# JADGardner/neusky

Hardware: AMD Instinct MI355X
Metric: train rays/sec on NeRF-OSR lk2 @1024 rays x 96 samples (higher is better)
Workload: dtype f32 in memory; forward products: fp16 hi + residual split, 3 x v_mfma_f32_32x32x16_f16 per product on power-of-two pre-scaled operands, one fp32 accumulator (~2^-22): FiLM-SIREN chains and the SDF / albedo field alike; backward products: the same fp16 split on per-row / per-matrix pre-scaled gradien; 1 GPU; full NeuSky train step (BASELINE configs[2]): 1024 rays/GPU x 96 samples, proposal 256+96, 512 illumination directions (256 upper-hemisphere DDF queries/ray), illumination decoder = this project's FiLM-SIREN H = 128 (RENI-shaped: latent 100x3; the reference's configured Attention decoder is absent from its tree), hash L16 F2 T2^19 x2, 256-wide MLPs; fwd + losses + bwd + all-reduce + 5 Adam groups; rays_per_gpu=1024, samples_per_ray=96, illumination_directions=512, parallelism=ray-sharded dp1, launcher=self-spawned, launch=HIP graph replay (1 graph/step + all-reduce + 5 Adam launches)

## Files before the change

### neusky_amd/csrc/field_chain.hip

```cpp
#include "chain.h"

namespace {

constexpr int H = 256, NT = 8, KS = 16;
constexpr int WAVES = 4, PW = 16 / WAVES, RG = WAVES == 8 ? 8 : 4, RING = RG * GROUP, THREADS = 64 * WAVES, WGS_PER_CU = 8 / WAVES;

struct ChainLayers { nsky_chain_layer l[NSKY_CHAIN_MAX_LAYERS]; int n; };

__host__ __device__ inline void chain_layout(const nsky_chain_layer* l, int n, long& groups, int& tiles) {
  groups = 0; tiles = 0;
  for (int i = 0; i < n; ++i) {
    const int t = (l[i].rows + 31) / 32;
    tiles += t;
    groups += (long)t * groups_of(l[i].K);
  }
}

__global__ __launch_bounds__(256) void chain_pack_kernel(ChainLayers L, unsigned char* __restrict__ stream, float* __restrict__ scales) {
  __shared__ float w[32][PACK_KMAX + 1];
  __shared__ float red[256];
  int tile = blockIdx.x, i = 0;
  long group = 0;
  for (; i < L.n; ++i) {
    const int t = (L.l[i].rows + 31) / 32;
    if (tile < t) break;
    tile -= t;
    group += (long)t * groups_of(L.l[i].K);
  }
  const nsky_chain_layer& y = L.l[i];
  TileDesc d;
  d.W = y.W; d.ld = y.ld; d.row0 = 32 * tile; d.nrows = min(32, y.rows - 32 * tile); d.K = y.K; d.transposed = y.transposed; d.k0 = 0;
  d.group = group + (long)tile * groups_of(y.K);
  pack_tile(d, stream, scales, w, red);
}

template <int G>
__device__ __forceinline__ float quad_bcast(float v) {
  return __int_as_float(__builtin_amdgcn_mov_dpp(__float_as_int(v), G * 0x55, 0xf, 0xf, true));
}
__device__ __forceinline__ float quad_bcast0(float v) { return quad_bcast<0>(v); }
__device__ __forceinline__ float quad_sum(float v) {
  v += __int_as_float(__builtin_amdgcn_mov_dpp(__float_as_int(v), 0xB1, 0xf, 0xf, true));
  v += __int_as_float(__builtin_amdgcn_mov_dpp(__float_as_int(v), 0x4E, 0xf, 0xf, true));
  return v;
}
__device__ __forceinline__ float quad_max(float v) {
  v = fmaxf(v, __int_as_float(__builtin_amdgcn_mov_dpp(__float_as_int(v), 0xB1, 0xf, 0xf, true)));
  v = fmaxf(v, __int_as_float(__builtin_amdgcn_mov_dpp(__float_as_int(v), 0x4E, 0xf, 0xf, true)));
  return v;
}
__device__ __forceinline__ void quad_scatter_value(const float (&x)[16], int j, float (&mine)[4]) {
#pragma unroll
// ... 625 lines not shown
  }
  for (int u = 0; u < ct; ++u) {
    f32x16 acc;
    prod<KS, PW, true, RG>(ws, ACTIVE, ph, pl, acc);
    if (ACTIVE && live && a.dET) {
      const float inv = p_inv * sl[NT + u];
      float* out = a.dET + ((long)j * a.N + n) * a.ldE;
#pragma unroll
      for (int g = 0; g < 4; ++g) {
        const int fo = 32 * u + 8 * g + 4 * h;
        if (fo < a.ldE) {
          float4 o = make_float4(acc[4 * g] * inv, acc[4 * g + 1] * inv, acc[4 * g + 2] * inv, acc[4 * g + 3] * inv);
          if (a.dxpe && j == 0 && fo < 40) {
            const float4 e = ldg4(a.dxpe + n * 40 + fo);
            o.x += e.x; o.y += e.y; o.z += e.z; o.w += e.w;
          }
          stg4(out + fo, o);
        }
      }
      asm volatile("s_waitcnt vmcnt(0)" ::: "memory");
    }
  }
}

__global__ __launch_bounds__(THREADS, 2) void field_geo_bwd_kernel(const GeoBwdArgs a) {
  __shared__ __attribute__((aligned(16))) unsigned char smem[RING + (H + 32) * 4];
  float* wl = reinterpret_cast<float*>(smem + RING);
  float* sl = wl + H;
  const int tid = threadIdx.x, lane = tid & 63;
  const int wave = __builtin_amdgcn_readfirstlane(tid >> 6);
  const int ct = (a.net.in_dim + 31) / 32;
  for (int i = tid; i < H; i += THREADS) wl[i] = a.net.w_sdf[i];
  for (int i = tid; i < NT + ct; i += THREADS) sl[i] = a.scales[i];
  __syncthreads();
  WStream ws;
  ws_open<PW, true, RG>(ws, a.stream, smem, wave, lane, a.total_groups);
  const long G = gridDim.x;
  for (long base = 0; base < a.n_tiles; base += WAVES * G) {
    const long tile = base + wave * G + blockIdx.x;
    if (tile < a.n_tiles) geo_bwd_tile<true>(a, ws, wl, sl, tile, lane, ct);
    else geo_bwd_tile<false>(a, ws, wl, sl, 0, lane, ct);
  }
  ws_close();
}

struct ColsumArgs {
  const float* X; int nt; int rows;
  const float* w4; int n_out;
  const float* g_sdf; const float* g_grad;
  float* out; int ldo; float* bias;
  int blocks_per_wg;
};

__global__ __launch_bounds__(512) void native_weighted_colsum_kernel(const ColsumArgs a) {
  const int tid = threadIdx.x, lane = tid & 63, wave = tid >> 6;
  const int c = lane & 31, h = lane >> 5;
  const int row_blocks = (a.rows + 31) / 32;
  const int b0 = blockIdx.x * a.blocks_per_wg, b1 = min(row_blocks, b0 + a.blocks_per_wg);
  for (int t = wave; t < a.nt; t += 8) {
    float acc[4][16];
    float bs[4] = {0.f, 0.f, 0.f, 0.f};
#pragma unroll
    for (int o = 0; o < 4; ++o)
#pragma unroll
      for (int r = 0; r < 16; ++r) acc[o][r] = 0.0f;
    for (int bb = b0; bb < b1; bb += 4) {
      float v[4][16], w[4][4];
#pragma unroll
      for (int u = 0; u < 4; ++u) {
        const int b = bb + u;
        const long row = (long)b * 32 + c;
        w[u][0] = w[u][1] = w[u][2] = w[u][3] = 0.0f;
        if (b < b1) {
          load_tile(a.X + ((long)b * a.nt + t) * 1024, lane, v[u]);
          if (row < a.rows) {
            if (a.w4) {
              const float4 q = ldg4(a.w4 + row * 4);
              w[u][0] = q.x; w[u][1] = q.y; w[u][2] = q.z; w[u][3] = q.w;
            } else {
              const int j = (int)(row & 3);
              const long n = row >> 2;
              w[u][0] = j == 0 ? (a.g_sdf ? a.g_sdf[n] : 0.0f) : (a.g_grad ? a.g_grad[n * 3 + (j - 1)] : 0.0f);
              if (j == 0) bs[0] += w[u][0];
            }
          }
        } else {
#pragma unroll
          for (int r = 0; r < 16; ++r) v[u][r] = 0.0f;
        }
      }
#pragma unroll
      for (int u = 0; u < 4; ++u) {
        if (a.w4) {
#pragma unroll
          for (int o = 0; o < 4; ++o) bs[o] += w[u][o];
        }
#pragma unroll
        for (int o = 0; o < 4; ++o)
          if (o < a.n_out)
#pragma unroll
            for (int r = 0; r < 16; ++r) acc[o][r] = fmaf(w[u][o], v[u][r], acc[o][r]);
      }
    }
#pragma unroll
    for (int o = 0; o < 4; ++o)
      if (o < a.n_out) {
#pragma unroll
        for (int r = 0; r < 16; ++r) {
          float v = acc[o][r];
#pragma unroll
          for (int off = 16; off > 0; off >>= 1) v += __shfl_xor(v, off, 64);
          if (c == 0 && v != 0.0f) atomicAdd(a.out + (long)o * a.ldo + 32 * t + 8 * (r >> 2) + 4 * h + (r & 3), v);
        }
        if (a.bias && t == 0) {
          float v = h == 0 ? bs[o] : 0.0f;
#pragma unroll
          for (int off = 16; off > 0; off >>= 1) v += __shfl_xor(v, off, 64);
          if (lane == 0 && v != 0.0f) atomicAdd(a.bias + o, v);
        }
      }
  }
}

int check_field_net(const nsky_field_net* n, const char* who) {
  NSKY_CHECK_ARG(n, "%s: null network", who);
  NSKY_CHECK_ARG(n->in_dim >= 4 && n->in_dim <= 80 && n->in_dim % 4 == 0 && n->npe >= 0 && n->npe <= 39 && n->beta > 0.0f,
                 "%s: in_dim %d (4..80, multiple of 4), npe %d (<= 39), beta %g", who, n->in_dim, n->npe, n->beta);
  return NSKY_OK;
}

int persistent_grid(int n_tiles) {
  const int cus = device_cus(), wgs = (n_tiles + WAVES - 1) / WAVES;
  return wgs < cus * WGS_PER_CU ? wgs : cus * WGS_PER_CU;
}

}

extern "C" int nsky_chain_stream_layout(const nsky_chain_layer* layers, int32_t n_layers, int64_t* stream_bytes, int32_t* n_tiles, int32_t* n_groups) {
  NSKY_CHECK_ARG(layers && n_layers >= 1 && n_layers <= NSKY_CHAIN_MAX_LAYERS, "nsky_chain_stream_layout: 1..%d layers", NSKY_CHAIN_MAX_LAYERS);
  for (int i = 0; i < n_layers; ++i)
    NSKY_CHECK_ARG(layers[i].rows >= 1 && layers[i].K >= 1 && layers[i].K <= PACK_KMAX, "nsky_chain_stream_layout: layer %d: rows %d, K %d (<= %d)", i,
                   layers[i].rows, layers[i].K, PACK_KMAX);
  long groups; int tiles;
  chain_layout(layers, n_layers, groups, tiles);
  if (stream_bytes) *stream_bytes = (groups + RING_GROUPS + 2) * (int64_t)GROUP;
  if (n_tiles) *n_tiles = tiles;
  if (n_groups) *n_groups = (int32_t)groups;
  return NSKY_OK;
}

extern "C" int nsky_chain_pack(const nsky_chain_layer* layers, int32_t n_layers, void* stream_buf, float* scales, nsky_stream_t stream) {
  if (int rc = nsky_chain_stream_layout(layers, n_layers, nullptr, nullptr, nullptr)) return rc;
  NSKY_CHECK_ARG(stream_buf && scales && ((uintptr_t)stream_buf % 16) == 0, "nsky_chain_pack: null / unaligned buffer");
  ChainLayers L;
  L.n = n_layers;
  for (int i = 0; i < n_layers; ++i) {
    L.l[i] = layers[i];
    NSKY_CHECK_ARG(L.l[i].W && L.l[i].ld >= (L.l[i].transposed ? L.l[i].rows : L.l[i].K), "nsky_chain_pack: layer %d: weights / ld", i);
  }
  long groups; int tiles;
  chain_layout(layers, n_layers, groups, tiles);
  hipLaunchKernelGGL(chain_pack_kernel, dim3(tiles), dim3(256), 0, (hipStream_t)stream, L, (unsigned char*)stream_buf, scales);
  NSKY_CHECK_LAUNCH("nsky_chain_pack");
  return NSKY_OK;
}

#define NSKY_AL16(p) (((uintptr_t)(p) % 16) == 0)

extern "C" int nsky_field_geo_fwd(const nsky_field_net* net, const void* stream_buf, const float* scales, int32_t total_groups, const float* ET,
                                  int32_t ldE, int32_t N, float* a0q, float* a1q, float* Eq, float* a1max, float* sdf, float* grad, float* qmax,
                                  nsky_stream_t stream) {
  if (int rc = check_field_net(net, "nsky_field_geo_fwd")) return rc;
  NSKY_CHECK_ARG(stream_buf && scales && ET && a0q && a1q && sdf && grad && N > 0 && net->b0 && net->b1 && net->w_sdf, "nsky_field_geo_fwd: null operand / empty batch");
// ... 19 lines not shown
  NSKY_CHECK_ARG(ldE % 4 == 0 && ldE >= net->npe + 1 && NSKY_AL16(ET) && NSKY_AL16(a1q) && NSKY_AL16(feat) && NSKY_AL16(xpe) && NSKY_AL16(c0) && NSKY_AL16(c1) && NSKY_AL16(alb) &&
                     (!a1v || NSKY_AL16(a1v)) && net->ldc2 >= H, "nsky_field_colour_fwd: alignment / leading dimensions");
  NSKY_CHECK_ARG(total_groups == NT * (2 * groups_of(H) + groups_of(300)), "nsky_field_colour_fwd: stream of %d groups does not hold W2f, Wc0, Wc1", total_groups);
  ColFwdArgs a;
  a.net = *net; a.stream = (const unsigned char*)stream_buf; a.scales = scales; a.total_groups = total_groups; a.ET = ET; a.ldE = ldE; a.N = N;
  a.n_tiles = ceil_div(N, 32); a.a1q = a1q; a.a1max = a1max; a.a1v = a1v; a.feat = feat; a.xpe = xpe; a.c0 = c0; a.c1 = c1; a.alb = alb;
  hipLaunchKernelGGL(field_colour_fwd_kernel, dim3(persistent_grid(a.n_tiles)), dim3(THREADS), 0, (hipStream_t)stream, a);
  NSKY_CHECK_LAUNCH("nsky_field_colour_fwd");
  return NSKY_OK;
}

extern "C" int nsky_field_colour_bwd(const nsky_field_net* net, const void* stream_buf, const float* scales, int32_t total_groups, int32_t N,
                                     const float* g_alb, const float* alb, const float* c0, const float* c1, float* dpc2, float* dpc1, float* dpc0,
                                     float* dfeat, float* dxpe, float* da1v, float* gmax, nsky_stream_t stream) {
  if (int rc = check_field_net(net, "nsky_field_colour_bwd")) return rc;
  NSKY_CHECK_ARG(stream_buf && scales && g_alb && alb && c0 && c1 && dpc2 && dpc1 && dpc0 && dfeat && da1v && gmax && N > 0 && net->wc2,
                 "nsky_field_colour_bwd: null operand / empty batch");
  NSKY_CHECK_ARG(NSKY_AL16(alb) && NSKY_AL16(c0) && NSKY_AL16(c1) && NSKY_AL16(dpc2) && NSKY_AL16(dpc1) && NSKY_AL16(dpc0) && NSKY_AL16(dfeat) && NSKY_AL16(da1v) &&
                     (!dxpe || NSKY_AL16(dxpe)) && net->ldc2 >= H, "nsky_field_colour_bwd: alignment");
  NSKY_CHECK_ARG(total_groups == (2 * NT + 10) * groups_of(H), "nsky_field_colour_bwd: stream of %d groups does not hold Wc1^T, Wc0^T, W2f^T", total_groups);
  ColBwdArgs a;
  a.net = *net; a.stream = (const unsigned char*)stream_buf; a.scales = scales; a.total_groups = total_groups; a.N = N; a.n_tiles = ceil_div(N, 32);
  a.g_alb = g_alb; a.alb = alb; a.c0 = c0; a.c1 = c1; a.dpc2 = dpc2; a.dpc1 = dpc1; a.dpc0 = dpc0; a.dfeat = dfeat; a.dxpe = dxpe; a.da1v = da1v; a.gmax = gmax;
  hipLaunchKernelGGL(field_colour_bwd_kernel, dim3(persistent_grid(a.n_tiles)), dim3(THREADS), 0, (hipStream_t)stream, a);
  NSKY_CHECK_LAUNCH("nsky_field_colour_bwd");
  return NSKY_OK;
}

extern "C" int nsky_field_geo_bwd(const nsky_field_net* net, const void* stream_buf, const float* scales, int32_t total_groups, int32_t N,
                                  const float* g_sdf, const float* g_grad, const float* da1v, const float* dxpe, const float* a0q, const float* a1q,
                                  float* d1q, float* d0q, float* dET, int32_t ldE, float* gmax, nsky_stream_t stream) {
  if (int rc = check_field_net(net, "nsky_field_geo_bwd")) return rc;
  NSKY_CHECK_ARG(stream_buf && scales && a0q && a1q && d1q && d0q && gmax && N > 0 && net->w_sdf, "nsky_field_geo_bwd: null operand / empty batch");
  NSKY_CHECK_ARG(NSKY_AL16(a0q) && NSKY_AL16(a1q) && NSKY_AL16(d1q) && NSKY_AL16(d0q) && (!da1v || NSKY_AL16(da1v)) && (!dxpe || NSKY_AL16(dxpe)) &&
                     (!dET || (NSKY_AL16(dET) && ldE % 4 == 0 && ldE >= net->in_dim)), "nsky_field_geo_bwd: alignment / ldE");
  const int ct = (net->in_dim + 31) / 32;
  NSKY_CHECK_ARG(total_groups == (NT + ct) * groups_of(H), "nsky_field_geo_bwd: stream of %d groups does not hold W1^T, W0^T", total_groups);
  GeoBwdArgs a;
  a.net = *net; a.stream = (const unsigned char*)stream_buf; a.scales = scales; a.total_groups = total_groups; a.N = N; a.n_tiles = ceil_div(N, 8);
  a.g_sdf = g_sdf; a.g_grad = g_grad; a.da1v = da1v; a.dxpe = dxpe; a.a0q = a0q; a.a1q = a1q; a.d1q = d1q; a.d0q = d0q; a.dET = dET; a.ldE = ldE; a.gmax = gmax;
  hipLaunchKernelGGL(field_geo_bwd_kernel, dim3(persistent_grid(a.n_tiles)), dim3(THREADS), 0, (hipStream_t)stream, a);
  NSKY_CHECK_LAUNCH("nsky_field_geo_bwd");
  return NSKY_OK;
}

extern "C" int nsky_native_weighted_colsum(const float* X, int32_t nt, int32_t rows, const float* w4, int32_t n_out, const float* g_sdf,
                                           const float* g_grad, float* out, int32_t ldo, float* bias, nsky_stream_t stream) {
  NSKY_CHECK_ARG(X && out && nt >= 1 && rows >= 0 && NSKY_AL16(X) && ldo >= 32 * nt, "nsky_native_weighted_colsum: bad argument");
  NSKY_CHECK_ARG(w4 ? (n_out >= 1 && n_out <= 4 && NSKY_AL16(w4)) : (n_out == 1 && rows % 4 == 0), "nsky_native_weighted_colsum: weights (n_out %d)", n_out);
  if (rows == 0) return NSKY_OK;
  ColsumArgs a;
  a.X = X; a.nt = nt; a.rows = rows; a.w4 = w4; a.n_out = n_out; a.g_sdf = g_sdf; a.g_grad = g_grad; a.out = out; a.ldo = ldo; a.bias = bias;
  const int row_blocks = ceil_div(rows, 32);
  a.blocks_per_wg = ceil_div(row_blocks, 256);
  hipLaunchKernelGGL(native_weighted_colsum_kernel, dim3(ceil_div(row_blocks, a.blocks_per_wg)), dim3(512), 0, (hipStream_t)stream, a);
  NSKY_CHECK_LAUNCH("nsky_native_weighted_colsum");
  return NSKY_OK;
}
```

### neusky_amd/csrc/samplers.hip

```cpp
#include "common.h"
#include "../../include/neusky_hip.h"

namespace {

constexpr float TWO_PI = 6.283185307179586f;

struct Philox {
  uint32_t k0, k1;
  __device__ __forceinline__ static void round(uint32_t (&c)[4], uint32_t k0, uint32_t k1) {
    const uint64_t p0 = (uint64_t)0xD2511F53u * c[0], p1 = (uint64_t)0xCD9E8D57u * c[2];
    const uint32_t n0 = (uint32_t)(p1 >> 32) ^ c[1] ^ k0, n1 = (uint32_t)p1, n2 = (uint32_t)(p0 >> 32) ^ c[3] ^ k1, n3 = (uint32_t)p0;
    c[0] = n0; c[1] = n1; c[2] = n2; c[3] = n3;
  }
  __device__ __forceinline__ void draw(uint32_t a, uint32_t b, uint64_t call, uint32_t (&out)[4]) const {
    uint32_t c[4] = {a, b, (uint32_t)call, (uint32_t)(call >> 32)};
    uint32_t x = k0, y = k1;
#pragma unroll
    for (int r = 0; r < 10; ++r) {
      round(c, x, y);
      x += 0x9E3779B9u;
      y += 0xBB67AE85u;
    }
#pragma unroll
    for (int i = 0; i < 4; ++i) out[i] = c[i];
  }
};

__device__ __forceinline__ float u01(uint32_t w) { return ((float)(w >> 9) + 0.5f) * (1.0f / 8388608.0f); }

__global__ void advance_counter_kernel(uint64_t* counter) { *counter += 1; }

__global__ __launch_bounds__(256) void ddf_vmf_samples_kernel(int n_pos, int n_dir, float kappa, float radius, int upper, uint64_t seed,
                                                              const uint64_t* __restrict__ counter, float* __restrict__ origins,
                                                              float* __restrict__ directions) {
  const int i = blockIdx.x * 256 + threadIdx.x;
  if (i >= n_pos * n_dir) return;
  const int n = i / n_dir;
  const uint64_t call = *counter;
  Philox rng{(uint32_t)seed, (uint32_t)(seed >> 32)};
  uint32_t w[4];
  rng.draw((uint32_t)n, 0u, call, w);
  const float theta = TWO_PI * u01(w[0]);
  const float cphi = 2.0f * u01(w[1]) - 1.0f;
  const float sphi = sqrtf(fmaxf(0.0f, 1.0f - cphi * cphi));
  float p[3] = {sphi * cosf(theta), sphi * sinf(theta), cphi};
  if (upper && p[2] < 0.0f) { p[0] = -p[0]; p[1] = -p[1]; p[2] = -p[2]; }
  const float nrm[3] = {-p[0], -p[1], -p[2]};
  rng.draw((uint32_t)i, 1u, call, w);
  const float r0 = sqrtf(-2.0f * logf(u01(w[0]))), r1 = sqrtf(-2.0f * logf(u01(w[2])));
  float z[3] = {r0 * cosf(TWO_PI * u01(w[1])), r0 * sinf(TWO_PI * u01(w[1])), r1 * cosf(TWO_PI * u01(w[3]))};
  float inv = rsqrtf(z[0] * z[0] + z[1] * z[1] + z[2] * z[2]);
  z[0] *= inv; z[1] *= inv; z[2] *= inv;
// ... 100 lines not shown
  float x[3], y[3], z[3];
  local_frame(pos, x, y, z);
  const float dl[3] = {x[0] * wd[0] + x[1] * wd[1] + x[2] * wd[2], y[0] * wd[0] + y[1] * wd[1] + y[2] * wd[2],
                       z[0] * wd[0] + z[1] * wd[1] + z[2] * wd[2]};
  float* row = a.xrow + (long)e * a.ldx;
  for (int c = 0; c < 3; ++c) { a.q_pos[(long)e * 3 + c] = pos[c]; row[c] = dl[c]; }
#pragma unroll
  for (int i = 0; i < 3; ++i)
#pragma unroll
    for (int f = 0; f < 2; ++f) {
      const float arg = TWO_PI * dl[i] * (f == 0 ? 1.0f : 4.0f);
      row[3 + i * 2 + f] = sinf(arg);
      row[9 + i * 2 + f] = sinf(arg + 1.5707963267948966f);
    }
  for (int c = 15; c < a.ldx; ++c) row[c] = 0.0f;
}

__global__ __launch_bounds__(256) void ddf_fit_rows_bwd_kernel(const float* __restrict__ positions, const float* __restrict__ directions,
                                                               const float* __restrict__ term_dist, const float* __restrict__ mv_points,
                                                               const float* __restrict__ d_xrow, int ldx, int N,
                                                               float* __restrict__ d_term_dist) {
  const int j = blockIdx.x * 256 + threadIdx.x;
  if (j >= N) return;
  const float pts[3] = {mv_points[j * 3], mv_points[j * 3 + 1], mv_points[j * 3 + 2]};
  const float t = term_dist[j];
  float dir[3], dv[3];
  for (int c = 0; c < 3; ++c) { dir[c] = directions[j * 3 + c]; dv[c] = positions[j * 3 + c] + dir[c] * t - pts[c]; }
  const float len = sqrtf(dv[0] * dv[0] + dv[1] * dv[1] + dv[2] * dv[2]);
  const float u[3] = {dv[0] / len, dv[1] / len, dv[2] / len};
  float x[3], y[3], z[3];
  local_frame(pts, x, y, z);
  const float dl[3] = {x[0] * u[0] + x[1] * u[1] + x[2] * u[2], y[0] * u[0] + y[1] * u[1] + y[2] * u[2], z[0] * u[0] + z[1] * u[1] + z[2] * u[2]};
  const float* g = d_xrow + (long)j * ldx;
  float gl[3];
#pragma unroll
  for (int i = 0; i < 3; ++i) {
    float acc = g[i];
#pragma unroll
    for (int f = 0; f < 2; ++f) {
      const float w = TWO_PI * (f == 0 ? 1.0f : 4.0f);
      const float arg = w * dl[i];
      acc += w * (g[3 + i * 2 + f] * cosf(arg) + g[9 + i * 2 + f] * cosf(arg + 1.5707963267948966f));
    }
    gl[i] = acc;
  }
  float gu[3];
  for (int c = 0; c < 3; ++c) gu[c] = x[c] * gl[0] + y[c] * gl[1] + z[c] * gl[2];
  const float ug = u[0] * gu[0] + u[1] * gu[1] + u[2] * gu[2];
  float gt = 0.0f;
  for (int c = 0; c < 3; ++c) gt += (gu[c] - u[c] * ug) / len * dir[c];
  d_term_dist[j] = gt;
}

__global__ __launch_bounds__(256) void reni_grid_inputs_fwd_kernel(const float* __restrict__ Z, const float* __restrict__ dirs, int U, int L,
                                                                   int D, const float* __restrict__ ray_dirs,
                                                                   const long* __restrict__ ray_latent, int R, float* __restrict__ cond,
                                                                   int ldc, float* __restrict__ xrow, int ldx) {
  const long t = (long)blockIdx.x * 256 + threadIdx.x;
  if (t >= ((long)U * D + R) * L) return;
  const int l = (int)(t % L);
  const long row = t / L;
  int u;
  const float* dp;
  if (row < (long)U * D) { u = (int)(row / D); dp = dirs + (row % D) * 3; }
  else { const long r = row - (long)U * D; u = (int)ray_latent[r]; dp = ray_dirs + r * 3; }
  const float zx = Z[((long)u * L + l) * 3], zy = Z[((long)u * L + l) * 3 + 1], zz = Z[((long)u * L + l) * 3 + 2];
  const float dx = dp[0], dy = dp[1];
  float* c = cond + row * ldc + 3 * l;
  c[0] = sqrtf(zx * zx + zy * zy);
  c[1] = zz;
  c[2] = zx * dx + zy * dy;
  if (l == 0) {
    for (int k = 3 * L; k < ldc; ++k) cond[row * ldc + k] = 0.0f;
    float* x = xrow + row * ldx;
    const float v[2] = {sqrtf(dx * dx + dy * dy), dp[2]};
    x[0] = v[0]; x[1] = v[1];
#pragma unroll
    for (int i = 0; i < 2; ++i)
#pragma unroll
      for (int f = 0; f < 2; ++f) {
        const float arg = TWO_PI * v[i] * (f == 0 ? 1.0f : 4.0f);
        x[2 + i * 2 + f] = sinf(arg);
        x[6 + i * 2 + f] = sinf(arg + 1.5707963267948966f);
      }
    for (int k = 10; k < ldx; ++k) x[k] = 0.0f;
  }
}

constexpr int RENI_BWD_ROWS = 32;
__global__ __launch_bounds__(320) void reni_grid_inputs_bwd_kernel(const float* __restrict__ Z, const float* __restrict__ dirs, int U, int L,
                                                                   int D, const float* __restrict__ d_cond, int ldc,
                                                                   float* __restrict__ d_Z) {
  const int u = blockIdx.y, d0 = blockIdx.x * RENI_BWD_ROWS;
  for (int col = threadIdx.x; col < 3 * L; col += blockDim.x) {
    const int l = col / 3, k = col % 3;
    float s0 = 0.f, s1 = 0.f;
#pragma unroll 8
    for (int j = 0; j < RENI_BWD_ROWS; ++j) {
      const int d = d0 + j;
      if (d < D) {
        const float g = d_cond[((long)u * D + d) * ldc + col];
        if (k == 2) { s0 = fmaf(g, dirs[d * 3], s0); s1 = fmaf(g, dirs[d * 3 + 1], s1); }
        else s0 += g;
      }
    }
    float* o = d_Z + ((long)u * L + l) * 3;
    if (k == 0) {
      const float zx = Z[((long)u * L + l) * 3], zy = Z[((long)u * L + l) * 3 + 1];
      const float n = sqrtf(zx * zx + zy * zy);
      if (n > 0.0f) { atomicAdd(o, s0 * zx / n); atomicAdd(o + 1, s0 * zy / n); }
    } else if (k == 1) {
      atomicAdd(o + 2, s0);
    } else {
      atomicAdd(o, s0); atomicAdd(o + 1, s1);
    }
  }
}

__global__ __launch_bounds__(256) void reni_ray_inputs_bwd_kernel(const float* __restrict__ Z, const float* __restrict__ ray_dirs,
                                                                  const long* __restrict__ ray_latent, int R, int L,
                                                                  const float* __restrict__ d_cond_rays, int ldc, float* __restrict__ d_Z) {
  const int t = blockIdx.x * 256 + threadIdx.x;
  if (t >= R * L) return;
  const int l = t % L, r = t / L;
  const long u = ray_latent[r];
  const float zx = Z[(u * L + l) * 3], zy = Z[(u * L + l) * 3 + 1];
  const float* g = d_cond_rays + (long)r * ldc + 3 * l;
  float gx = g[2] * ray_dirs[r * 3], gy = g[2] * ray_dirs[r * 3 + 1];
  const float n = sqrtf(zx * zx + zy * zy);
  if (n > 0.0f) { gx += g[0] * zx / n; gy += g[0] * zy / n; }
  float* o = d_Z + (u * L + l) * 3;
  atomicAdd(o, gx); atomicAdd(o + 1, gy); atomicAdd(o + 2, g[1]);
}

__global__ __launch_bounds__(256) void grid_probe_points_kernel(const float* __restrict__ lattice, float gx, float gy, float gz, int P, uint64_t seed,
                                                                const uint64_t* __restrict__ counter, float* __restrict__ pos,
                                                                float* __restrict__ dirs) {
  const int p = blockIdx.x * 256 + threadIdx.x;
  if (p >= P) return;
  const Philox g{(uint32_t)seed, (uint32_t)(seed >> 32)};
  uint32_t a[4], b[4];
  g.draw(0x47524944u, (uint32_t)p, *counter, a);
  g.draw(0x47524945u, (uint32_t)p, *counter, b);
  pos[3 * p] = lattice[3 * p] + (u01(a[0]) * gx - 0.5f * gx);
  pos[3 * p + 1] = lattice[3 * p + 1] + (u01(a[1]) * gy - 0.5f * gy);
  pos[3 * p + 2] = lattice[3 * p + 2] + (u01(a[2]) * gz - 0.5f * gz);
  const float r0 = sqrtf(-2.0f * logf(u01(b[0]))), r1 = sqrtf(-2.0f * logf(u01(b[2])));
  const float x = r0 * cosf(TWO_PI * u01(b[1])), y = r0 * sinf(TWO_PI * u01(b[1])), z = r1 * cosf(TWO_PI * u01(b[3]));
  const float inv = 1.0f / sqrtf(x * x + y * y + z * z);
  dirs[3 * p] = x * inv; dirs[3 * p + 1] = y * inv; dirs[3 * p + 2] = z * inv;
}

__global__ __launch_bounds__(256) void reni_output_fwd_kernel(const float* __restrict__ raw, int ldr, const float* __restrict__ scale,
                                                              const long* __restrict__ ray_latent, int U, int D, int R,
                                                              float* __restrict__ grid, float* __restrict__ rays) {
  const int i = blockIdx.x * 256 + threadIdx.x;
  if (i >= U * D + R) return;
  const float s = scale[i < U * D ? i / D : ray_latent[i - U * D]];
  float* o = i < U * D ? grid + 3l * i : rays + 3l * (i - U * D);
#pragma unroll
  for (int c = 0; c < 3; ++c) o[c] = expf(raw[(long)i * ldr + c]) * s;
}

__global__ __launch_bounds__(256) void reni_output_bwd_kernel(const float* __restrict__ raw, int ldr, const float* __restrict__ scale,
                                                              const long* __restrict__ ray_latent, int U, int D, int R,
                                                              const float* __restrict__ d_grid, const float* __restrict__ d_rays,
                                                              float* __restrict__ d_raw, float* __restrict__ d_scale) {
  const int i = blockIdx.x * 256 + threadIdx.x;
// ... 83 lines not shown
  for (int w = 0; w < wave; ++w) before += wave_total[w];
  if (chosen) sel[before + __popcll(mask & ((1ull << lane) - 1ull))] = t;
}

}

extern "C" int nsky_ddf_vmf_samples(int32_t n_positions, int32_t n_directions, float kappa, float radius, int32_t upper_hemisphere,
                                    uint64_t seed, uint64_t* counter, float* origins, float* directions, nsky_stream_t stream) {
  NSKY_CHECK_ARG(n_positions >= 0 && n_directions >= 0 && counter && kappa > 0.0f, "nsky_ddf_vmf_samples: bad argument");
  const long n = (long)n_positions * n_directions;
  if (n == 0) return NSKY_OK;
  NSKY_CHECK_ARG(origins && directions, "nsky_ddf_vmf_samples: null output");
  hipLaunchKernelGGL(ddf_vmf_samples_kernel, dim3(ceil_div(n, 256)), dim3(256), 0, (hipStream_t)stream, n_positions, n_directions, kappa,
                     radius, upper_hemisphere, seed, counter, origins, directions);
  hipLaunchKernelGGL(advance_counter_kernel, dim3(1), dim3(1), 0, (hipStream_t)stream, counter);
  NSKY_CHECK_LAUNCH("nsky_ddf_vmf_samples");
  return NSKY_OK;
}

extern "C" int nsky_ddf_fit_rows_fwd(const float* positions, const float* directions, const float* term_dist, int32_t N,
                                     const float* mv_points_in, uint64_t seed, uint64_t* counter, const float* sky_o, const float* sky_d,
                                     int32_t Ns, float radius, int32_t want_mv, float weight_exp, int32_t weight_include_z, float* q_pos,
                                     float* xrow, int32_t ldx, float* mv_points_out, float* sky_gt, float* distance_weight,
                                     nsky_stream_t stream) {
  NSKY_CHECK_ARG(N >= 0 && Ns >= 0 && ldx >= 15 && radius > 0.0f, "nsky_ddf_fit_rows_fwd: bad sizes");
  const int n_mv = want_mv ? N : 0;
  const int E = N + n_mv + Ns;
  if (E == 0) return NSKY_OK;
  NSKY_CHECK_ARG(q_pos && xrow && (N == 0 || (positions && directions)) && (n_mv == 0 || (term_dist && mv_points_out)) &&
                     (Ns == 0 || (sky_o && sky_d && sky_gt)), "nsky_ddf_fit_rows_fwd: null argument");
  NSKY_CHECK_ARG(n_mv == 0 || mv_points_in || counter, "nsky_ddf_fit_rows_fwd: multi-view points are neither given nor can they be drawn (no counter)");
  FitRowsArgs a;
  a.positions = positions; a.directions = directions; a.term_dist = term_dist; a.mv_in = mv_points_in; a.sky_o = sky_o; a.sky_d = sky_d;
  a.counter = counter; a.seed = seed; a.q_pos = q_pos; a.xrow = xrow; a.mv_out = mv_points_out; a.sky_gt = sky_gt;
  a.dist_weight = distance_weight; a.N = N; a.Ns = Ns; a.ldx = ldx; a.want_mv = want_mv; a.include_z = weight_include_z;
  a.radius = radius; a.weight_exp = weight_exp;
  hipLaunchKernelGGL(ddf_fit_rows_fwd_kernel, dim3(ceil_div(E, 256)), dim3(256), 0, (hipStream_t)stream, a);
  if (n_mv > 0 && !mv_points_in) hipLaunchKernelGGL(advance_counter_kernel, dim3(1), dim3(1), 0, (hipStream_t)stream, counter);
  NSKY_CHECK_LAUNCH("nsky_ddf_fit_rows_fwd");
  return NSKY_OK;
}

extern "C" int nsky_ddf_fit_rows_bwd(const float* positions, const float* directions, const float* term_dist, const float* mv_points,
                                     int32_t N, const float* d_xrow_mv, int32_t ldx, float* d_term_dist, nsky_stream_t stream) {
  if (N == 0) return NSKY_OK;
  NSKY_CHECK_ARG(positions && directions && term_dist && mv_points && d_xrow_mv && d_term_dist && N > 0 && ldx >= 15,
                 "nsky_ddf_fit_rows_bwd: bad argument");
  hipLaunchKernelGGL(ddf_fit_rows_bwd_kernel, dim3(ceil_div(N, 256)), dim3(256), 0, (hipStream_t)stream, positions, directions, term_dist,
                     mv_points, d_xrow_mv, ldx, N, d_term_dist);
  NSKY_CHECK_LAUNCH("nsky_ddf_fit_rows_bwd");
  return NSKY_OK;
}

extern "C" int nsky_reni_grid_inputs_fwd(const float* latents, const float* directions, int32_t U, int32_t L, int32_t D,
                                         const float* ray_dirs, const int64_t* ray_latent, int32_t R, float* cond, int32_t ldcond,
                                         float* xrow, int32_t ldx, nsky_stream_t stream) {
  const long n = ((long)U * D + R) * L;
  if (n == 0) return NSKY_OK;
  NSKY_CHECK_ARG(latents && cond && xrow && ldcond >= 3 * L && ldx >= 10 && (D == 0 || directions) && (R == 0 || (ray_dirs && ray_latent)),
                 "nsky_reni_grid_inputs_fwd: bad argument");
  hipLaunchKernelGGL(reni_grid_inputs_fwd_kernel, dim3(ceil_div(n, 256)), dim3(256), 0, (hipStream_t)stream, latents, directions, U, L, D,
                     ray_dirs, reinterpret_cast<const long*>(ray_latent), R, cond, ldcond, xrow, ldx);
  NSKY_CHECK_LAUNCH("nsky_reni_grid_inputs_fwd");
  return NSKY_OK;
}

extern "C" int nsky_reni_grid_inputs_bwd(const float* latents, const float* directions, int32_t U, int32_t L, int32_t D,
                                         const float* ray_dirs, const int64_t* ray_latent, int32_t R, const float* d_cond, int32_t ldcond,
                                         float* d_latents, nsky_stream_t stream) {
  if ((long)U * L == 0) return NSKY_OK;
  NSKY_CHECK_ARG(latents && d_cond && d_latents && ldcond >= 3 * L && (D == 0 || directions) && (R == 0 || (ray_dirs && ray_latent)),
                 "nsky_reni_grid_inputs_bwd: bad argument");
  if (hipMemsetAsync(d_latents, 0, sizeof(float) * 3 * (size_t)U * L, (hipStream_t)stream) != hipSuccess) {
    nsky_set_error("nsky_reni_grid_inputs_bwd: memset failed");
    return NSKY_ERR_LAUNCH;
  }
  if (D > 0)
    hipLaunchKernelGGL(reni_grid_inputs_bwd_kernel, dim3(ceil_div(D, RENI_BWD_ROWS), U), dim3(320), 0, (hipStream_t)stream, latents,
                       directions, U, L, D, d_cond, ldcond, d_latents);
  if (R > 0)
    hipLaunchKernelGGL(reni_ray_inputs_bwd_kernel, dim3(ceil_div((long)R * L, 256)), dim3(256), 0, (hipStream_t)stream, latents, ray_dirs,
                       reinterpret_cast<const long*>(ray_latent), R, L, d_cond + (long)U * D * ldcond, ldcond, d_latents);
  NSKY_CHECK_LAUNCH("nsky_reni_grid_inputs_bwd");
  return NSKY_OK;
}

extern "C" int nsky_illumination_directions(const float* base, int32_t D, const float* rotation_in, uint64_t seed, uint64_t* counter, float* dirs,
                                            int32_t* sel, float* rot_out, nsky_stream_t stream) {
  NSKY_CHECK_ARG(base && dirs && sel && D >= 2 && D <= 1024 && D % 2 == 0 && (rotation_in || counter),
                 "nsky_illumination_directions: bad argument (D %d: even, <= 1024)", D);
  hipLaunchKernelGGL(illumination_directions_kernel, dim3(1), dim3((D + 63) / 64 * 64), 0, (hipStream_t)stream, base, D, rotation_in, seed, counter,
                     dirs, sel, rot_out);
  NSKY_CHECK_LAUNCH("nsky_illumination_directions");
  return NSKY_OK;
}

extern "C" int nsky_reni_output_fwd(const float* raw, int32_t ldr, const float* scale, const int64_t* ray_latent, int32_t U, int32_t D, int32_t R,
                                    float* grid, float* rays, nsky_stream_t stream) {
  NSKY_CHECK_ARG(raw && scale && ldr >= 3 && U >= 0 && D >= 0 && R >= 0 && (U * D == 0 || grid) && (R == 0 || (rays && ray_latent)),
                 "nsky_reni_output_fwd: bad argument");
  const int n = U * D + R;
  if (n == 0) return NSKY_OK;
  hipLaunchKernelGGL(reni_output_fwd_kernel, dim3(ceil_div(n, 256)), dim3(256), 0, (hipStream_t)stream, raw, ldr, scale, (const long*)ray_latent, U, D,
                     R, grid, rays);
  NSKY_CHECK_LAUNCH("nsky_reni_output_fwd");
  return NSKY_OK;
}

extern "C" int nsky_reni_output_bwd(const float* raw, int32_t ldr, const float* scale, const int64_t* ray_latent, int32_t U, int32_t D, int32_t R,
                                    const float* d_grid, const float* d_rays, float* d_raw, float* d_scale, nsky_stream_t stream) {
  NSKY_CHECK_ARG(raw && scale && d_raw && ldr >= 3 && ldr <= 4 && U >= 0 && D >= 0 && R >= 0 && (R == 0 || ray_latent), "nsky_reni_output_bwd: bad argument");
  const int n = U * D + R;
  if (n == 0) return NSKY_OK;
  hipLaunchKernelGGL(reni_output_bwd_kernel, dim3(ceil_div(n, 256)), dim3(256), 0, (hipStream_t)stream, raw, ldr, scale, (const long*)ray_latent, U, D,
                     R, d_grid, d_rays, d_raw, d_scale);
  NSKY_CHECK_LAUNCH("nsky_reni_output_bwd");
  return NSKY_OK;
}

extern "C" int nsky_grid_probe_points(const float* lattice, const float* gap3_host, int32_t P, uint64_t seed, uint64_t* counter, float* positions,
                                      float* directions, nsky_stream_t stream) {
  if (P == 0) return NSKY_OK;
  NSKY_CHECK_ARG(lattice && gap3_host && counter && positions && directions && P > 0, "nsky_grid_probe_points: bad argument");
  hipLaunchKernelGGL(grid_probe_points_kernel, dim3(ceil_div(P, 256)), dim3(256), 0, (hipStream_t)stream, lattice, gap3_host[0], gap3_host[1],
                     gap3_host[2], P, seed, counter, positions, directions);
  hipLaunchKernelGGL(advance_counter_kernel, dim3(1), dim3(1), 0, (hipStream_t)stream, counter);
  NSKY_CHECK_LAUNCH("nsky_grid_probe_points");
  return NSKY_OK;
}
```

Baseline: 50980 rays/s.

## Restructure weighted colsum and RENI input kernels with LDS staging and templating

The weighted column-sum kernel is templated on output count and moved to 4-wave blocks. Weights are staged in LDS and several waves share each tile, with partial sums reduced through LDS instead of per-lane shuffles and atomics, and the per-workgroup block count is sized to the CU count. The RENI grid-input forward kernel now stages latents and directions per row block in LDS and writes vectorised float4 rows. The backward kernel reduces over direction slices in LDS and writes directly when a single slice exists, which skips the memset and atomics. These kernels are small parts of a large train step, so the effect on the whole step is likely small, and the new code adds more synchronisation plus a limit of 256 latents per set.

```diff
diff --git a/neusky_amd/csrc/field_chain.hip b/neusky_amd/csrc/field_chain.hip
--- a/neusky_amd/csrc/field_chain.hip
+++ b/neusky_amd/csrc/field_chain.hip
@@ -1,3 +1,4 @@
+#include <algorithm>
 #include "chain.h"
 
 namespace {
@@ -729,73 +730,98 @@
   int blocks_per_wg;
 };
 
-__global__ __launch_bounds__(512) void native_weighted_colsum_kernel(const ColsumArgs a) {
-  const int tid = threadIdx.x, lane = tid & 63, wave = tid >> 6;
-  const int c = lane & 31, h = lane >> 5;
+constexpr int CS_WAVES = 4, CS_BLOCKS = 32;
+
+template <int N_OUT>
+__global__ __launch_bounds__(64 * CS_WAVES) void native_weighted_colsum_kernel(const ColsumArgs a) {
+  __shared__ float4 wl[CS_BLOCKS * 32];
+  __shared__ float red[CS_WAVES * 16 * 64];
+  const int tid = threadIdx.x, lane = tid & 63;
+  const int wave = __builtin_amdgcn_readfirstlane(tid >> 6);
+  const int c = lane & 31;
   const int row_blocks = (a.rows + 31) / 32;
   const int b0 = blockIdx.x * a.blocks_per_wg, b1 = min(row_blocks, b0 + a.blocks_per_wg);
-  for (int t = wave; t < a.nt; t += 8) {
-    float acc[4][16];
-    float bs[4] = {0.f, 0.f, 0.f, 0.f};
-#pragma unroll
-    for (int o = 0; o < 4; ++o)
+  float bs[4] = {0.f, 0.f, 0.f, 0.f};
+  for (int i = tid; i < (b1 - b0) * 32; i += 64 * CS_WAVES) {
+    const long row = (long)b0 * 32 + i;
+    float4 q = make_float4(0.f, 0.f, 0.f, 0.f);
+    bool in_bias = false;
+    if (row < a.rows) {
+      if (a.w4) {
+        q = ldg4(a.w4 + row * 4);
+        in_bias = true;
+      } else {
+        const int j = (int)(row & 3);
+        const long n = row >> 2;
+        q.x = j == 0 ? (a.g_sdf ? a.g_sdf[n] : 0.0f) : (a.g_grad ? a.g_grad[n * 3 + (j - 1)] : 0.0f);
+        in_bias = j == 0;
+      }
+    }
+    wl[i] = q;
+    if (in_bias) { bs[0] += q.x; bs[1] += q.y; bs[2] += q.z; bs[3] += q.w; }
+  }
+  if (a.bias) {
+#pragma unroll
+    for (int o = 0; o < N_OUT; ++o) {
+      float v = bs[o];
+#pragma unroll
+      for (int off = 32; off > 0; off >>= 1) v += __shfl_xor(v, off, 64);
+      if (lane == 0 && v != 0.0f) atomicAdd(a.bias + o, v);
+    }
+  }
+  const int slots = min(a.nt, CS_WAVES), wpc = CS_WAVES / slots;
+  const int cs = wave / wpc, sub = wave - cs * wpc;
+  for (int t0 = 0; t0 < a.nt; t0 += slots) {
+    const int t = t0 + cs;
+    const bool on = cs < slots && t < a.nt;
+    float acc[N_OUT][16];
+#pragma unroll
+    for (int o = 0; o < N_OUT; ++o)
 #pragma unroll
       for (int r = 0; r < 16; ++r) acc[o][r] = 0.0f;
-    for (int bb = b0; bb < b1; bb += 4) {
-      float v[4][16], w[4][4];
-#pragma unroll
-      for (int u = 0; u < 4; ++u) {
-        const int b = bb + u;
-        const long row = (long)b * 32 + c;
-        w[u][0] = w[u][1] = w[u][2] = w[u][3] = 0.0f;
-        if (b < b1) {
-          load_tile(a.X + ((long)b * a.nt + t) * 1024, lane, v[u]);
-          if (row < a.rows) {
-            if (a.w4) {
-              const float4 q = ldg4(a.w4 + row * 4);
-              w[u][0] = q.x; w[u][1] = q.y; w[u][2] = q.z; w[u][3] = q.w;
-            } else {
-              const int j = (int)(row & 3);
-              const long n = row >> 2;
-              w[u][0] = j == 0 ? (a.g_sdf ? a.g_sdf[n] : 0.0f) : (a.g_grad ? a.g_grad[n * 3 + (j - 1)] : 0.0f);
-              if (j == 0) bs[0] += w[u][0];
-            }
-          }
-        } else {
-#pragma unroll
-          for (int r = 0; r < 16; ++r) v[u][r] = 0.0f;
-        }
-      }
-#pragma unroll
-      for (int u = 0; u < 4; ++u) {
-        if (a.w4) {
-#pragma unroll
-          for (int o = 0; o < 4; ++o) bs[o] += w[u][o];
-        }
-#pragma unroll
-        for (int o = 0; o < 4; ++o)
-          if (o < a.n_out)
-#pragma unroll
-            for (int r = 0; r < 16; ++r) acc[o][r] = fmaf(w[u][o], v[u][r], acc[o][r]);
-      }
-    }
-#pragma unroll
-    for (int o = 0; o < 4; ++o)
-      if (o < a.n_out) {
-#pragma unroll
-        for (int r = 0; r < 16; ++r) {
-          float v = acc[o][r];
-#pragma unroll
-          for (int off = 16; off > 0; off >>= 1) v += __shfl_xor(v, off, 64);
-          if (c == 0 && v != 0.0f) atomicAdd(a.out + (long)o * a.ldo + 32 * t + 8 * (r >> 2) + 4 * h + (r & 3), v);
-        }
-        if (a.bias && t == 0) {
-          float v = h == 0 ? bs[o] : 0.0f;
-#pragma unroll
-          for (int off = 16; off > 0; off >>= 1) v += __shfl_xor(v, off, 64);
-          if (lane == 0 && v != 0.0f) atomicAdd(a.bias + o, v);
-        }
-      }
+    __syncthreads();
+    if (on) {
+      float va[4][16];
+      const float* xt = a.X + (long)t * 1024;
+      const long pitch = (long)a.nt * 1024;
+      auto issue = [&](float (&v)[4][16], int bb) {
+#pragma unroll
+        for (int u = 0; u < 4; ++u) load_tile(xt + min(bb + u * wpc, b1 - 1) * pitch, lane, v[u]);
+      };
+      auto consume = [&](const float (&v)[4][16], int bb) {
+#pragma unroll
+        for (int u = 0; u < 4; ++u) {
+          const int b = bb + u * wpc;
+          const float4 q = wl[(min(b, b1 - 1) - b0) * 32 + c];
+          const float m = b < b1 ? 1.0f : 0.0f;
+          const float w[4] = {q.x * m, q.y * m, q.z * m, q.w * m};
+#pragma unroll
+          for (int o = 0; o < N_OUT; ++o)
+#pragma unroll
+            for (int r = 0; r < 16; ++r) acc[o][r] = fmaf(w[o], v[u][r], acc[o][r]);
+        }
+      };
+      const int step = 4 * wpc;
+      for (int bb = b0 + sub; bb < b1; bb += step) {
+        issue(va, bb);
+        consume(va, bb);
+      }
+    }
+#pragma unroll
+    for (int o = 0; o < N_OUT; ++o) {
+      if (o > 0) __syncthreads();
+#pragma unroll
+      for (int r = 0; r < 16; ++r) red[(wave * 16 + r) * 64 + lane] = acc[o][r];
+      __syncthreads();
+      if (tid < slots * 32) {
+        const int s2 = tid >> 5, r = (tid >> 1) & 15, h = tid & 1;
+        float v = 0.0f;
+        for (int w = 0; w < wpc; ++w)
+#pragma unroll 8
+          for (int k = 0; k < 32; ++k) v += red[((s2 * wpc + w) * 16 + r) * 64 + h * 32 + ((k + tid) & 31)];
+        if (t0 + s2 < a.nt && v != 0.0f) atomicAdd(a.out + (long)o * a.ldo + 32 * (t0 + s2) + 8 * (r >> 2) + 4 * h + (r & 3), v);
+      }
+    }
   }
 }
 
@@ -921,8 +947,14 @@
   ColsumArgs a;
   a.X = X; a.nt = nt; a.rows = rows; a.w4 = w4; a.n_out = n_out; a.g_sdf = g_sdf; a.g_grad = g_grad; a.out = out; a.ldo = ldo; a.bias = bias;
   const int row_blocks = ceil_div(rows, 32);
-  a.blocks_per_wg = ceil_div(row_blocks, 256);
-  hipLaunchKernelGGL(native_weighted_colsum_kernel, dim3(ceil_div(row_blocks, a.blocks_per_wg)), dim3(512), 0, (hipStream_t)stream, a);
+  a.blocks_per_wg = std::min(CS_BLOCKS, std::max(1, ceil_div(row_blocks, 2 * device_cus())));
+  const dim3 grid(ceil_div(row_blocks, a.blocks_per_wg)), block(64 * CS_WAVES);
+  switch (n_out) {
+    case 1: hipLaunchKernelGGL(native_weighted_colsum_kernel<1>, grid, block, 0, (hipStream_t)stream, a); break;
+    case 2: hipLaunchKernelGGL(native_weighted_colsum_kernel<2>, grid, block, 0, (hipStream_t)stream, a); break;
+    case 3: hipLaunchKernelGGL(native_weighted_colsum_kernel<3>, grid, block, 0, (hipStream_t)stream, a); break;
+    default: hipLaunchKernelGGL(native_weighted_colsum_kernel<4>, grid, block, 0, (hipStream_t)stream, a); break;
+  }
   NSKY_CHECK_LAUNCH("nsky_native_weighted_colsum");
   return NSKY_OK;
 }
diff --git a/neusky_amd/csrc/samplers.hip b/neusky_amd/csrc/samplers.hip
--- a/neusky_amd/csrc/samplers.hip
+++ b/neusky_amd/csrc/samplers.hip
@@ -1,3 +1,4 @@
+#include <algorithm>
 #include "common.h"
 #include "../../include/neusky_hip.h"
 
@@ -204,68 +205,146 @@
   d_term_dist[j] = gt;
 }
 
+constexpr int RENI_MAX_L = 256;
+constexpr int RENI_FWD_ROWS = 64, RENI_RAY_ROWS = 8;
+
+__device__ __forceinline__ float reni_norm_zxy(float zx, float zy) {
+#pragma clang fp contract(off)
+  return sqrtf(fmaf(zx, zx, zy * zy));
+}
+__device__ __forceinline__ float reni_dot_xy(float zx, float zy, float dx, float dy) {
+#pragma clang fp contract(off)
+  return fmaf(zx, dx, zy * dy);
+}
+__device__ __forceinline__ float reni_norm_dxy(float dx, float dy) {
+#pragma clang fp contract(off)
+  return sqrtf(dx * dx + dy * dy);
+}
+__device__ __forceinline__ float reni_xrow_value(int k, float dx, float dy, float dz) {
+#pragma clang fp contract(off)
+  if (k >= 10) return 0.0f;
+  const int i = k < 2 ? k : ((k - 2) >> 1) & 1;
+  const float v = i == 0 ? reni_norm_dxy(dx, dy) : dz;
+  if (k < 2) return v;
+  const float arg = TWO_PI * v * (((k - 2) & 1) == 0 ? 1.0f : 4.0f);
+  return k < 6 ? sinf(arg) : sinf(arg + 1.5707963267948966f);
+}
+
+template <bool VEC>
 __global__ __launch_bounds__(256) void reni_grid_inputs_fwd_kernel(const float* __restrict__ Z, const float* __restrict__ dirs, int U, int L,
                                                                    int D, const float* __restrict__ ray_dirs,
                                                                    const long* __restrict__ ray_latent, int R, float* __restrict__ cond,
-                                                                   int ldc, float* __restrict__ xrow, int ldx) {
-  const long t = (long)blockIdx.x * 256 + threadIdx.x;
-  if (t >= ((long)U * D + R) * L) return;
-  const int l = (int)(t % L);
-  const long row = t / L;
-  int u;
-  const float* dp;
-  if (row < (long)U * D) { u = (int)(row / D); dp = dirs + (row % D) * 3; }
-  else { const long r = row - (long)U * D; u = (int)ray_latent[r]; dp = ray_dirs + r * 3; }
-  const float zx = Z[((long)u * L + l) * 3], zy = Z[((long)u * L + l) * 3 + 1], zz = Z[((long)u * L + l) * 3 + 2];
-  const float dx = dp[0], dy = dp[1];
-  float* c = cond + row * ldc + 3 * l;
-  c[0] = sqrtf(zx * zx + zy * zy);
-  c[1] = zz;
-  c[2] = zx * dx + zy * dy;
-  if (l == 0) {
-    for (int k = 3 * L; k < ldc; ++k) cond[row * ldc + k] = 0.0f;
-    float* x = xrow + row * ldx;
-    const float v[2] = {sqrtf(dx * dx + dy * dy), dp[2]};
-    x[0] = v[0]; x[1] = v[1];
-#pragma unroll
-    for (int i = 0; i < 2; ++i)
-#pragma unroll
-      for (int f = 0; f < 2; ++f) {
-        const float arg = TWO_PI * v[i] * (f == 0 ? 1.0f : 4.0f);
-        x[2 + i * 2 + f] = sinf(arg);
-        x[6 + i * 2 + f] = sinf(arg + 1.5707963267948966f);
+                                                                   int ldc, float* __restrict__ xrow, int ldx, int grid_wgs_per_set) {
+  extern __shared__ __attribute__((aligned(16))) float reni_lds[];
+  float4* zs = reinterpret_cast<float4*>(reni_lds);
+  const int tid = threadIdx.x;
+  const bool rays = (int)blockIdx.x >= U * grid_wgs_per_set;
+  long row0;
+  int n_rows;
+  if (!rays) {
+    const int u = blockIdx.x / grid_wgs_per_set, d0 = (blockIdx.x % grid_wgs_per_set) * RENI_FWD_ROWS;
+    row0 = (long)u * D + d0;
+    n_rows = min(RENI_FWD_ROWS, D - d0);
+  } else {
+    const int r0 = (blockIdx.x - U * grid_wgs_per_set) * RENI_RAY_ROWS;
+    row0 = (long)U * D + r0;
+    n_rows = min(RENI_RAY_ROWS, R - r0);
+  }
+  const int n_sets = rays ? n_rows : 1;
+  float* dxyz = reni_lds + 4 * RENI_RAY_ROWS * L;
+  for (int i = tid; i < n_sets * L; i += 256) {
+    const int s = i / L, l = i - s * L;
+    const long u = rays ? ray_latent[row0 - (long)U * D + s] : row0 / D;
+    const float* z = Z + (u * L + l) * 3;
+    zs[i] = make_float4(z[0], z[1], z[2], reni_norm_zxy(z[0], z[1]));
+  }
+  {
+    const float* src = rays ? ray_dirs + (row0 - (long)U * D) * 3 : dirs + (row0 % D) * 3;
+    for (int i = tid; i < 3 * n_rows; i += 256) dxyz[i] = src[i];
+  }
+  __syncthreads();
+  const int pc = VEC ? ldc / 4 : ldc;
+  for (int i = tid; i < n_rows * pc; i += 256) {
+    const int r = i / pc, p = i - r * pc;
+    const float4* zr = zs + (rays ? r * L : 0);
+    const float dx = dxyz[3 * r], dy = dxyz[3 * r + 1];
+    float v[4];
+#pragma unroll
+    for (int j = 0; j < (VEC ? 4 : 1); ++j) {
+      const int c = (VEC ? 4 * p : p) + j;
+      const int l = c / 3, k = c - 3 * l;
+      float val = 0.0f;
+      if (c < 3 * L) {
+        const float4 z = zr[l];
+        val = k == 0 ? z.w : k == 1 ? z.z : reni_dot_xy(z.x, z.y, dx, dy);
       }
-    for (int k = 10; k < ldx; ++k) x[k] = 0.0f;
-  }
-}
-
-constexpr int RENI_BWD_ROWS = 32;
-__global__ __launch_bounds__(320) void reni_grid_inputs_bwd_kernel(const float* __restrict__ Z, const float* __restrict__ dirs, int U, int L,
+      v[j] = val;
+    }
+    float* o = cond + (row0 + r) * ldc;
+    if (VEC) *reinterpret_cast<float4*>(o + 4 * p) = make_float4(v[0], v[1], v[2], v[3]);
+    else o[p] = v[0];
+  }
+  const int px = VEC ? ldx / 4 : ldx;
+  for (int i = tid; i < n_rows * px; i += 256) {
+    const int r = i / px, p = i - r * px;
+    const float dx = dxyz[3 * r], dy = dxyz[3 * r + 1], dz = dxyz[3 * r + 2];
+    float* o = xrow + (row0 + r) * ldx;
+    if (VEC) *reinterpret_cast<float4*>(o + 4 * p) = make_float4(reni_xrow_value(4 * p, dx, dy, dz), reni_xrow_value(4 * p + 1, dx, dy, dz),
+                                                                reni_xrow_value(4 * p + 2, dx, dy, dz), reni_xrow_value(4 * p + 3, dx, dy, dz));
+    else o[p] = reni_xrow_value(p, dx, dy, dz);
+  }
+}
+
+constexpr int RENI_BWD_SLICE = 256;
+template <bool VEC>
+__global__ __launch_bounds__(256) void reni_grid_inputs_bwd_kernel(const float* __restrict__ Z, const float* __restrict__ dirs, int U, int L,
                                                                    int D, const float* __restrict__ d_cond, int ldc,
-                                                                   float* __restrict__ d_Z) {
-  const int u = blockIdx.y, d0 = blockIdx.x * RENI_BWD_ROWS;
-  for (int col = threadIdx.x; col < 3 * L; col += blockDim.x) {
-    const int l = col / 3, k = col % 3;
-    float s0 = 0.f, s1 = 0.f;
-#pragma unroll 8
-    for (int j = 0; j < RENI_BWD_ROWS; ++j) {
-      const int d = d0 + j;
-      if (d < D) {
-        const float g = d_cond[((long)u * D + d) * ldc + col];
-        if (k == 2) { s0 = fmaf(g, dirs[d * 3], s0); s1 = fmaf(g, dirs[d * 3 + 1], s1); }
-        else s0 += g;
-      }
-    }
+                                                                   float* __restrict__ d_Z, int slice_rows) {
+  __shared__ float dxy[RENI_BWD_SLICE * 2];
+  __shared__ float red[256 * 12];
+  __shared__ float col[RENI_MAX_L * 3 * 3];
+  const int tid = threadIdx.x;
+  const int u = blockIdx.y, d0 = blockIdx.x * slice_rows, d1 = min(D, d0 + slice_rows);
+  const int Q = (3 * L + 3) / 4, G = 256 / Q;
+  for (int i = tid; i < d1 - d0; i += 256) { dxy[2 * i] = dirs[(d0 + i) * 3]; dxy[2 * i + 1] = dirs[(d0 + i) * 3 + 1]; }
+  __syncthreads();
+  const int g = tid / Q, q = tid - g * Q;
+  float s[4] = {0.f, 0.f, 0.f, 0.f}, sx[4] = {0.f, 0.f, 0.f, 0.f}, sy[4] = {0.f, 0.f, 0.f, 0.f};
+  if (g < G) {
+    const float* base = d_cond + ((long)u * D) * ldc + 4 * q;
+#pragma unroll 4
+    for (int d = d0 + g; d < d1; d += G) {
+      const float* p = base + (long)d * ldc;
+      float4 v;
+      if (VEC) v = *reinterpret_cast<const float4*>(p);
+      else v = make_float4(p[0], 4 * q + 1 < 3 * L ? p[1] : 0.0f, 4 * q + 2 < 3 * L ? p[2] : 0.0f, 4 * q + 3 < 3 * L ? p[3] : 0.0f);
+      const float dx = dxy[2 * (d - d0)], dy = dxy[2 * (d - d0) + 1];
+      const float e[4] = {v.x, v.y, v.z, v.w};
+#pragma unroll
+      for (int j = 0; j < 4; ++j) { s[j] += e[j]; sx[j] = fmaf(e[j], dx, sx[j]); sy[j] = fmaf(e[j], dy, sy[j]); }
+    }
+  }
+#pragma unroll
+  for (int j = 0; j < 4; ++j) { red[(j * 3 + 0) * 256 + tid] = s[j]; red[(j * 3 + 1) * 256 + tid] = sx[j]; red[(j * 3 + 2) * 256 + tid] = sy[j]; }
+  __syncthreads();
+  for (int i = tid; i < 3 * L * 3; i += 256) {
+    const int c = i / 3, w = i - 3 * c;
+    float acc = 0.0f;
+    for (int gg = 0; gg < G; ++gg) acc += red[((c & 3) * 3 + w) * 256 + gg * Q + (c >> 2)];
+    col[i] = acc;
+  }
+  __syncthreads();
+  for (int l = tid; l < L; l += 256) {
+    const float* z = Z + ((long)u * L + l) * 3;
+    const float zx = z[0], zy = z[1];
+    const float n = sqrtf(zx * zx + zy * zy);
+    float gx = col[(3 * l + 2) * 3 + 1], gy = col[(3 * l + 2) * 3 + 2];
+    const float s0 = col[(3 * l) * 3];
+    if (n > 0.0f) { gx += s0 * zx / n; gy += s0 * zy / n; }
+    const float gz = col[(3 * l + 1) * 3];
     float* o = d_Z + ((long)u * L + l) * 3;
-    if (k == 0) {
-      const float zx = Z[((long)u * L + l) * 3], zy = Z[((long)u * L + l) * 3 + 1];
-      const float n = sqrtf(zx * zx + zy * zy);
-      if (n > 0.0f) { atomicAdd(o, s0 * zx / n); atomicAdd(o + 1, s0 * zy / n); }
-    } else if (k == 1) {
-      atomicAdd(o + 2, s0);
-    } else {
-      atomicAdd(o, s0); atomicAdd(o + 1, s1);
-    }
+    if (gridDim.x == 1) { o[0] = gx; o[1] = gy; o[2] = gz; }
+    else { atomicAdd(o, gx); atomicAdd(o + 1, gy); atomicAdd(o + 2, gz); }
   }
 }
 
@@ -455,6 +534,8 @@
   return NSKY_OK;
 }
 
+#define NSKY_RENI_VEC(p, ld) (((uintptr_t)(p) % 16) == 0 && (ld) % 4 == 0)
+
 extern "C" int nsky_reni_grid_inputs_fwd(const float* latents, const float* directions, int32_t U, int32_t L, int32_t D,
                                          const float* ray_dirs, const int64_t* ray_latent, int32_t R, float* cond, int32_t ldcond,
                                          float* xrow, int32_t ldx, nsky_stream_t stream) {
@@ -462,8 +543,16 @@
   if (n == 0) return NSKY_OK;
   NSKY_CHECK_ARG(latents && cond && xrow && ldcond >= 3 * L && ldx >= 10 && (D == 0 || directions) && (R == 0 || (ray_dirs && ray_latent)),
                  "nsky_reni_grid_inputs_fwd: bad argument");
-  hipLaunchKernelGGL(reni_grid_inputs_fwd_kernel, dim3(ceil_div(n, 256)), dim3(256), 0, (hipStream_t)stream, latents, directions, U, L, D,
-                     ray_dirs, reinterpret_cast<const long*>(ray_latent), R, cond, ldcond, xrow, ldx);
+  NSKY_CHECK_ARG(L <= RENI_MAX_L, "nsky_reni_grid_inputs_fwd: %d latents per set (at most %d)", L, RENI_MAX_L);
+  const int per_set = ceil_div(D, RENI_FWD_ROWS);
+  const dim3 grid(U * per_set + ceil_div(R, RENI_RAY_ROWS));
+  const size_t lds = sizeof(float) * (4 * RENI_RAY_ROWS * (size_t)L + 3 * RENI_FWD_ROWS);
+  if (NSKY_RENI_VEC(cond, ldcond) && NSKY_RENI_VEC(xrow, ldx) && ldx >= 12)
+    hipLaunchKernelGGL(reni_grid_inputs_fwd_kernel<true>, grid, dim3(256), lds, (hipStream_t)stream, latents, directions, U, L, D, ray_dirs,
+                       reinterpret_cast<const long*>(ray_latent), R, cond, ldcond, xrow, ldx, per_set);
+  else
+    hipLaunchKernelGGL(reni_grid_inputs_fwd_kernel<false>, grid, dim3(256), lds, (hipStream_t)stream, latents, directions, U, L, D, ray_dirs,
+                       reinterpret_cast<const long*>(ray_latent), R, cond, ldcond, xrow, ldx, per_set);
   NSKY_CHECK_LAUNCH("nsky_reni_grid_inputs_fwd");
   return NSKY_OK;
 }
@@ -474,13 +563,25 @@
   if ((long)U * L == 0) return NSKY_OK;
   NSKY_CHECK_ARG(latents && d_cond && d_latents && ldcond >= 3 * L && (D == 0 || directions) && (R == 0 || (ray_dirs && ray_latent)),
                  "nsky_reni_grid_inputs_bwd: bad argument");
-  if (hipMemsetAsync(d_latents, 0, sizeof(float) * 3 * (size_t)U * L, (hipStream_t)stream) != hipSuccess) {
+  NSKY_CHECK_ARG(L <= RENI_MAX_L, "nsky_reni_grid_inputs_bwd: %d latents per set (at most %d)", L, RENI_MAX_L);
+  int slices = 1, slice_rows = D;
+  if (D > 0) {
+    slices = std::max(std::min(ceil_div(1024, U), ceil_div(D, 32)), ceil_div(D, RENI_BWD_SLICE));
+    slice_rows = ceil_div(D, slices);
+    slices = ceil_div(D, slice_rows);
+  }
+  if ((D == 0 || slices > 1) && hipMemsetAsync(d_latents, 0, sizeof(float) * 3 * (size_t)U * L, (hipStream_t)stream) != hipSuccess) {
     nsky_set_error("nsky_reni_grid_inputs_bwd: memset failed");
     return NSKY_ERR_LAUNCH;
   }
-  if (D > 0)
-    hipLaunchKernelGGL(reni_grid_inputs_bwd_kernel, dim3(ceil_div(D, RENI_BWD_ROWS), U), dim3(320), 0, (hipStream_t)stream, latents,
-                       directions, U, L, D, d_cond, ldcond, d_latents);
+  if (D > 0) {
+    if (NSKY_RENI_VEC(d_cond, ldcond))
+      hipLaunchKernelGGL(reni_grid_inputs_bwd_kernel<true>, dim3(slices, U), dim3(256), 0, (hipStream_t)stream, latents, directions, U, L, D,
+                         d_cond, ldcond, d_latents, slice_rows);
+    else
+      hipLaunchKernelGGL(reni_grid_inputs_bwd_kernel<false>, dim3(slices, U), dim3(256), 0, (hipStream_t)stream, latents, directions, U, L, D,
+                         d_cond, ldcond, d_latents, slice_rows);
+  }
   if (R > 0)
     hipLaunchKernelGGL(reni_ray_inputs_bwd_kernel, dim3(ceil_div((long)R * L, 256)), dim3(256), 0, (hipStream_t)stream, latents, ray_dirs,
                        reinterpret_cast<const long*>(ray_latent), R, L, d_cond + (long)U * D * ldcond, ldcond, d_latents);
```

Result: no change. 51190 rays/s (median of 6 runs) (+0.4%).
